# Hypersonic-cpu/DSP-AudioRecLabs

Hardware: NVIDIA B200
Metric: audio-seconds processed/sec (features+endpoints+KNN) (higher is better)
Workload: dtype i16->f32/f64

## Files before the change

dsp_audioreclabs_b200/csrc/capi.cu:

```cuda
#include <cmath>
#include <cstdarg>
#include <cstdio>
#include <cstdlib>
#include <cstring>
#include <string>
#include <vector>

#include "kernels.cuh"
#include "knn.cuh"
#include "mfcc_dtw.cuh"
#include "misc.cuh"

using namespace dsp;

namespace {

thread_local std::string g_err;

int fail(int code, const char* fmt, ...) {
  char buf[512];
  va_list ap;
  va_start(ap, fmt);
  vsnprintf(buf, sizeof buf, fmt, ap);
  va_end(ap);
// ... 779 lines not shown
  if (rc) return rc;
  CU(cudaMemcpyAsync(mean, dm, sizeof(double) * d, cudaMemcpyDeviceToHost, c->stream));
  CU(cudaMemcpyAsync(std, ds, sizeof(double) * d, cudaMemcpyDeviceToHost, c->stream));
  if (out) CU(cudaMemcpyAsync(out, dy, sizeof(double) * (size_t)n * d, cudaMemcpyDeviceToHost, c->stream));
  CU(cudaStreamSynchronize(c->stream));
  return DSP_OK;
}

static void knn_release(dsp_knn* k) {
  DevBuf* all[] = {&k->train64, &k->train32, &k->labels, &k->tnorm, &k->cand_idx, &k->cand_worst, &k->qnorm,
                   &k->redo_list, &k->redo_count, &k->nbr_label, &k->q, &k->o_idx, &k->o_dist, &k->o_lab,
                   &k->tpacked, &k->tnorm_dense, &k->qpacked, &k->qnorm_chunk, &k->dense_flags, &k->part_d, &k->part_i,
                   &k->tc_train, &k->tc_train_rows, &k->tc_q, &k->tc_flags, &k->refine_list, &k->refine_thr, &k->surv_count, &k->surv_rows, &k->thr0,
                   &k->prune_perm, &k->prune_geom, &k->prune_box, &k->prune_ws, &k->prune_bound};
  for (DevBuf* b : all) b->release();
}

int dsp_knn_fit_device(dsp_context* c, const double* train, const int32_t* labels, int64_t n, int32_t d, int32_t k,
                       int64_t index_base, dsp_knn** out) {
  if (!c || !out || n < 1 || d < 1 || k < 1 || !train || !labels) return fail(DSP_ERR_INVALID, "bad argument");
  if (k > kKnnMaxK) return fail(DSP_ERR_UNSUPPORTED, "n_neighbors > %d is not supported", kKnnMaxK);
  if (n > INT32_MAX) return fail(DSP_ERR_UNSUPPORTED, "more than 2^31 train rows per shard");
  CU(cudaSetDevice(c->device));
  dsp_knn* h = new dsp_knn();
  h->ctx = c; h->n = n; h->d = d; h->k = k; h->index_base = index_base; h->dp = knn_padded_dim(d);
  auto bail = [&](int code) { knn_release(h); delete h; return code; };
  if (h->train64.ensure(sizeof(double) * (size_t)n * d) != cudaSuccess || h->labels.ensure(sizeof(int32_t) * (size_t)n) != cudaSuccess ||
      h->tnorm.ensure(64) != cudaSuccess || h->redo_count.ensure(64) != cudaSuccess)
    return bail(fail(DSP_ERR_NOMEM, "device allocation failed"));
  cudaMemcpyAsync(h->train64.p, train, sizeof(double) * (size_t)n * d, cudaMemcpyDeviceToDevice, c->stream);
  cudaMemcpyAsync(h->labels.p, labels, sizeof(int32_t) * (size_t)n, cudaMemcpyDeviceToDevice, c->stream);
  if (h->dp) {
    if (h->train32.ensure(sizeof(float) * (size_t)n * h->dp) != cudaSuccess) return bail(fail(DSP_ERR_NOMEM, "device allocation failed"));
    cudaError_t e = knn_pack(h->train64.as<double>(), n, d, h->dp, h->train32.as<float>(), h->tnorm.as<float>(), c->stream);
    c->launches++;
    if (e != cudaSuccess) return bail(fail(DSP_ERR_CUDA, "knn_pack: %s", cudaGetErrorString(e)));
    cudaMemcpyAsync(&h->tnorm_max, h->tnorm.p, sizeof(float), cudaMemcpyDeviceToHost, c->stream);
  }
  int tc_flags[2] = {0, 1};
  if (h->dp == 16 && n >= 64 && k < kKnnCand && std::getenv("DSP_KNN_NO_TC16") == nullptr) {
    std::vector<double> host((size_t)n * d);
    if (cudaMemcpyAsync(host.data(), h->train64.p, sizeof(double) * host.size(), cudaMemcpyDeviceToHost, c->stream) != cudaSuccess ||
        cudaStreamSynchronize(c->stream) != cudaSuccess)
      return bail(fail(DSP_ERR_CUDA, "knn fit: %s", cudaGetErrorString(cudaGetLastError())));
    KnnPrunePlan plan;
    knn_prune_plan(host.data(), n, d, plan);
    h->prune_tiles = (int64_t)plan.slack.size();
    const size_t box = sizeof(double) * plan.lo.size();
    if (h->tc_train.ensure(knn_tc16_packed_bytes(n, false)) != cudaSuccess || h->tc_flags.ensure(64) != cudaSuccess ||
        h->prune_perm.ensure(sizeof(int) * (size_t)n) != cudaSuccess || h->prune_geom.ensure(sizeof(KnnPruneGeom)) != cudaSuccess ||
        h->prune_box.ensure(2 * box + sizeof(double) * plan.slack.size()) != cudaSuccess)
      return bail(fail(DSP_ERR_NOMEM, "device allocation failed"));
    unsigned char* pb = h->prune_box.as<unsigned char>();
    cudaMemcpyAsync(h->prune_perm.p, plan.perm.data(), sizeof(int) * (size_t)n, cudaMemcpyHostToDevice, c->stream);
    cudaMemcpyAsync(h->prune_geom.p, &plan.geom, sizeof(KnnPruneGeom), cudaMemcpyHostToDevice, c->stream);
    cudaMemcpyAsync(pb, plan.lo.data(), box, cudaMemcpyHostToDevice, c->stream);
    cudaMemcpyAsync(pb + box, plan.hi.data(), box, cudaMemcpyHostToDevice, c->stream);
    cudaMemcpyAsync(pb + 2 * box, plan.slack.data(), sizeof(double) * plan.slack.size(), cudaMemcpyHostToDevice, c->stream);
    if (h->tc_train_rows.ensure(knn_tc16_packed_bytes(n, false)) != cudaSuccess) return bail(fail(DSP_ERR_NOMEM, "device allocation failed"));
    cudaError_t e = knn_tc16_pack(h->train64.as<double>(), n, d, false, h->tc_train_rows.p, nullptr, h->tc_flags.as<int>(), c->stream);
    if (e == cudaSuccess)
      e = knn_tc16_pack(h->train64.as<double>(), n, d, false, h->tc_train.p, nullptr, h->tc_flags.as<int>(), c->stream,
                        h->prune_perm.as<int>());
    c->launches++;
    if (e != cudaSuccess) return bail(fail(DSP_ERR_CUDA, "knn_tc16_pack: %s", cudaGetErrorString(e)));
    cudaMemcpyAsync(tc_flags, h->tc_flags.p, sizeof tc_flags, cudaMemcpyDeviceToHost, c->stream);
    if (cudaStreamSynchronize(c->stream) != cudaSuccess)
      return bail(fail(DSP_ERR_CUDA, "knn fit: %s", cudaGetErrorString(cudaGetLastError())));
  }
  int dense_flags[2] = {0, 0};
  if (!h->dp && d <= kKnnDenseMaxDim && std::getenv("DSP_KNN_NO_DENSE") == nullptr) {
    if (h->tpacked.ensure(knn_dense_packed_bytes(n, d, true)) != cudaSuccess ||
        h->tnorm_dense.ensure(sizeof(float) * (size_t)knn_dense_padded_rows(n, true)) != cudaSuccess ||
        h->dense_flags.ensure(64) != cudaSuccess)
      return bail(fail(DSP_ERR_NOMEM, "device allocation failed"));
    cudaError_t e = knn_dense_pack(h->train64.as<double>(), n, d, true, h->tpacked.p, h->tnorm_dense.as<float>(), INFINITY,
                                   h->dense_flags.as<int>(), true, c->stream);
    c->launches++;
    if (e != cudaSuccess) return bail(fail(DSP_ERR_CUDA, "knn_dense_pack: %s", cudaGetErrorString(e)));
    cudaMemcpyAsync(dense_flags, h->dense_flags.p, sizeof dense_flags, cudaMemcpyDeviceToHost, c->stream);
  }
  cudaError_t e = cudaStreamSynchronize(c->stream);
  if (e != cudaSuccess) return bail(fail(DSP_ERR_CUDA, "knn fit: %s", cudaGetErrorString(e)));
  h->tc16 = h->tc_train.p && tc_flags[1] == 0;
  if (h->tpacked.p) {
    std::memcpy(&h->tnorm_max, &dense_flags[0], sizeof(float));
    h->dense = dense_flags[1] == 0;
  }
  *out = h;
  return DSP_OK;
}

int dsp_knn_fit_host(dsp_context* c, const double* train, const int32_t* labels, int64_t n, int32_t d, int32_t k,
                     int64_t index_base, dsp_knn** out) {
  if (!c || !out || n < 1 || d < 1 || k < 1 || !train || !labels) return fail(DSP_ERR_INVALID, "bad argument");
  if (k > kKnnMaxK) return fail(DSP_ERR_UNSUPPORTED, "n_neighbors > %d is not supported", kKnnMaxK);
  CU(cudaSetDevice(c->device));
  OneShot os(c);
  double* dt = os.dev<double>((size_t)n * d);
  int32_t* dl = os.dev<int32_t>((size_t)n);
  if (!dt || !dl) return fail(DSP_ERR_NOMEM, "device allocation failed");
  CU(cudaMemcpyAsync(dt, train, sizeof(double) * (size_t)n * d, cudaMemcpyHostToDevice, c->stream));
  CU(cudaMemcpyAsync(dl, labels, sizeof(int32_t) * (size_t)n, cudaMemcpyHostToDevice, c->stream));
  return dsp_knn_fit_device(c, dt, dl, n, d, k, index_base, out);
}

int dsp_knn_free(dsp_knn* k) {
  if (!k) return DSP_OK;
  cudaSetDevice(k->ctx->device);
  cudaStreamSynchronize(k->ctx->stream);
  knn_release(k);
  delete k;
  return DSP_OK;
}

int dsp_knn_topk_device(dsp_knn* h, const double* q, int64_t m, int64_t* nbr_idx, double* nbr_sqdist, int32_t* nbr_label) {
  return dsp_knn_topk_bounded_device(h, q, m, nullptr, nbr_idx, nbr_sqdist, nbr_label);
}

int dsp_knn_topk_bounded_device(dsp_knn* h, const double* q, int64_t m, const double* bound, int64_t* nbr_idx, double* nbr_sqdist,
                                int32_t* nbr_label) {
  if (!h || m < 0 || (!q && m)) return fail(DSP_ERR_INVALID, "bad argument");
  if (m == 0) return DSP_OK;
  if (m > INT32_MAX) return fail(DSP_ERR_UNSUPPORTED, "more than 2^31 queries per call");
  dsp_context* c = h->ctx;
  CU(cudaSetDevice(c->device));
  CU(h->redo_list.ensure(sizeof(int32_t) * (size_t)m));
  const unsigned long long* prune_kept = nullptr;
  int64_t prune_visits = 0;
  if (h->dp) {
    CU(h->cand_idx.ensure(sizeof(int) * (size_t)m * kKnnCand));
    CU(h->cand_worst.ensure(sizeof(float) * (size_t)m));
    CU(h->qnorm.ensure(sizeof(float) * (size_t)m));
    double err_rel = (double)(h->d + 4) * 1.1920929e-7, err_floor = 0.0;
    float qnorm_limit = 0.f;
    const float* thr0 = nullptr;
    const double* rerank_bound = nullptr;
    if (h->tc16) {
      CU(h->tc_q.ensure(knn_tc16_packed_bytes(m, true)));
      int* qflags = h->tc_flags.as<int>() + 4;
      err_rel = knn_dense_err_rel(16);
      err_floor = 1.0;
      qnorm_limit = knn_tc16_max_norm();
      Tc16Work work;
      const void* tpacked = h->tc_train_rows.p;
      const bool prune = c->knn_prune && knn_tc16_padded_rows(m, true) / kTc16UnitQueries * h->prune_tiles <= INT32_MAX;
      if (prune) {
        CU(h->prune_ws.ensure(knn_prune_scratch_bytes(m, h->n)));
        CU(h->prune_bound.ensure(sizeof(double) * (size_t)m));
        CU(h->thr0.ensure(sizeof(float) * (size_t)m));
        const unsigned char* pb = h->prune_box.as<unsigned char>();
        const size_t box = sizeof(double) * (size_t)h->prune_tiles * h->d;
        CU(knn_prune_prepare(q, m, h->n, h->d, h->k, h->train64.as<double>(), h->prune_geom.as<KnnPruneGeom>(), h->prune_perm.as<int>(),
                             (const double*)pb, (const double*)(pb + box), (const double*)(pb + 2 * box), h->tc_train.p, h->tc_q.p,
                             h->qnorm.as<float>(), qflags, bound, h->prune_bound.as<double>(), h->cand_idx.as<int>(),
                             h->cand_worst.as<float>(), h->prune_ws.p, c->knn_prune == 1, c->sm_count, c->stream, work));
        tpacked = h->tc_train.p;
        rerank_bound = h->prune_bound.as<double>();
        prune_kept = work.kept;
        prune_visits = knn_tc16_padded_rows(m, true) / kTc16UnitQueries * h->prune_tiles;
        CU(knn_bound_thresholds(rerank_bound, h->qnorm.as<float>(), m, err_rel, err_floor, h->thr0.as<float>(), c->stream));
        thr0 = h->thr0.as<float>();
        c->launches += 12;
      } else {
        CU(knn_tc16_pack(q, m, h->d, true, h->tc_q.p, h->qnorm.as<float>(), qflags, c->stream));
      }
      if (bound && !prune) {
        CU(h->thr0.ensure(sizeof(float) * (size_t)m));
        CU(knn_bound_thresholds(bound, h->qnorm.as<float>(), m, err_rel, err_floor, h->thr0.as<float>(), c->stream));
        thr0 = h->thr0.as<float>();
        rerank_bound = bound;
        c->launches += 1;
      }
      CU(knn_tc16_filter(h->tc_q.p, tpacked, m, h->n, h->k, qflags, h->cand_idx.as<int>(), h->cand_worst.as<float>(),
                         c->sm_count, c->stream, thr0, work));
      c->launches += 2;
    } else {
      CU(knn_scan(h->dp, h->train32.as<float>(), h->n, q, m, h->d, h->cand_idx.as<int>(), h->cand_worst.as<float>(),
                  h->qnorm.as<float>(), nullptr, c->stream));
      c->launches += 1;
    }
    const int refine_cap = (h->dp == 16 && h->k < kKnnCand) ? (int)std::min<int64_t>(m, 65536) : 0;
    h->refine_cap = refine_cap;
    if (refine_cap) {
      CU(h->refine_list.ensure(sizeof(int32_t) * (size_t)refine_cap));
      CU(h->refine_thr.ensure(sizeof(float) * (size_t)refine_cap));
      CU(h->surv_count.ensure(sizeof(int32_t) * (size_t)refine_cap));
      CU(h->surv_rows.ensure(sizeof(int32_t) * (size_t)refine_cap * knn_refine_survivor_cap()));
    }
    CU(knn_rerank(h->train64.as<double>(), h->train32.as<float>(), h->dp, h->n, q, m, h->d, h->k, h->index_base,
                  h->labels.as<int32_t>(), h->cand_idx.as<int>(), h->cand_worst.as<float>(), h->qnorm.as<float>(),
                  h->tnorm_max, err_rel, err_floor, nbr_idx, nbr_sqdist, nbr_label, h->redo_list.as<int32_t>(),
                  h->redo_count.as<int32_t>(), c->stream, refine_cap ? h->refine_list.as<int32_t>() : nullptr,
                  h->refine_thr.as<float>(), refine_cap, qnorm_limit, rerank_bound, thr0, bound && thr0));
    c->launches += 1;
    if (refine_cap) {
      CU(knn_refine(h->train64.as<double>(), h->train32.as<float>(), h->dp, h->n, q, h->d, h->k, h->index_base,
                    h->labels.as<int32_t>(), h->refine_list.as<int32_t>(), h->refine_thr.as<float>(), refine_cap,
                    h->surv_count.as<int32_t>(), h->surv_rows.as<int32_t>(), h->redo_count.as<int32_t>(),
                    h->redo_list.as<int32_t>(), nbr_idx, nbr_sqdist, nbr_label, c->sm_count, c->stream, bound && thr0));
      c->launches += 2;
    }
  } else if (h->dense) {
    h->refine_cap = 0;
    CU(h->cand_idx.ensure(sizeof(int) * (size_t)m * kKnnCand));
    CU(h->cand_worst.ensure(sizeof(float) * (size_t)m));
    CU(h->qnorm.ensure(sizeof(float) * (size_t)m));
    const int64_t chunk = std::min<int64_t>(m, kKnnDenseQueryChunk);
    CU(h->qpacked.ensure(knn_dense_packed_bytes(chunk, h->d, false)));
    CU(h->qnorm_chunk.ensure(sizeof(float) * (size_t)knn_dense_padded_rows(chunk, false)));
    CU(h->dense_flags.ensure(64));
    for (int64_t q0 = 0; q0 < m; q0 += chunk) {
      const int64_t mc = std::min<int64_t>(chunk, m - q0);
      CU(knn_dense_pack(q + q0 * h->d, mc, h->d, false, h->qpacked.p, h->qnorm_chunk.as<float>(), 0.f, h->dense_flags.as<int>(),
                        q0 == 0, c->stream));
      CU(cudaMemcpyAsync(h->qnorm.as<float>() + q0, h->qnorm_chunk.p, sizeof(float) * (size_t)mc, cudaMemcpyDeviceToDevice, c->stream));
      CU(knn_dense_scan(h->qpacked.p, h->tpacked.p, h->tnorm_dense.as<float>(), mc, h->n, h->d,
                        h->cand_idx.as<int>() + q0 * kKnnCand, h->cand_worst.as<float>() + q0, c->sm_count, c->stream));
      c->launches += 2;
    }
    int qflags[2] = {0, 0};
    CU(cudaMemcpyAsync(qflags, h->dense_flags.p, sizeof qflags, cudaMemcpyDeviceToHost, c->stream));
    CU(cudaStreamSynchronize(c->stream));
    const bool all_fit = qflags[1] == 0;
    if (all_fit) {
      CU(knn_rerank(h->train64.as<double>(), nullptr, 0, h->n, q, m, h->d, h->k, h->index_base,
                    h->labels.as<int32_t>(), h->cand_idx.as<int>(), h->cand_worst.as<float>(), h->qnorm.as<float>(),
                    h->tnorm_max, knn_dense_err_rel(h->d), 0.0, nbr_idx, nbr_sqdist, nbr_label, h->redo_list.as<int32_t>(),
                    h->redo_count.as<int32_t>(), c->stream));
    } else {
      CU(knn_redo_all(h->redo_list.as<int32_t>(), h->redo_count.as<int32_t>(), m, c->stream));
    }
    c->launches++;
  } else {
    h->refine_cap = 0;
    CU(knn_redo_all(h->redo_list.as<int32_t>(), h->redo_count.as<int32_t>(), m, c->stream));
    c->launches++;
  }
  CU(h->part_d.ensure(sizeof(double) * (size_t)knn_rescan_grid(c->sm_count) * kKnnMaxK));
  CU(h->part_i.ensure(sizeof(long long) * (size_t)knn_rescan_grid(c->sm_count) * kKnnMaxK));
  CU(knn_rescan(h->train64.as<double>(), h->n, q, h->d, h->k, h->index_base, h->labels.as<int32_t>(),
                h->redo_list.as<int32_t>(), h->redo_count.as<int32_t>(), nbr_idx, nbr_sqdist, nbr_label,
                c->sm_count, h->part_d.as<double>(), h->part_i.as<long long>(), (int)std::min<int64_t>(m, INT32_MAX), c->stream));
  c->launches++;
  if (std::getenv("DSP_KNN_DEBUG")) {
    int32_t cnt[4];
    cudaMemcpyAsync(cnt, h->redo_count.p, sizeof cnt, cudaMemcpyDeviceToHost, c->stream);
    cudaStreamSynchronize(c->stream);
    fprintf(stderr, "[knn] m=%lld n=%lld exhaustive=%d refined=%d refined->exhaustive=%d\n", (long long)m, (long long)h->n, cnt[0],
            std::min(cnt[1], h->refine_cap), cnt[2]);
    if (prune_kept) {
      unsigned long long kept = 0;
      cudaMemcpyAsync(&kept, prune_kept, sizeof kept, cudaMemcpyDeviceToHost, c->stream);
      cudaStreamSynchronize(c->stream);
      fprintf(stderr, "[knn] prune: tile visits kept=%llu of %lld (%s)\n", kept, (long long)prune_visits,
              c->knn_prune == 1 && kept > (unsigned long long)(0.85 * (double)prune_visits) ? "every tile walked" : "lists walked");
    }
  }
  return DSP_OK;
}

int dsp_mfcc_batch_host(dsp_context* c, const int16_t* samples, const int64_t* offsets, const int32_t* lengths,
                        const int32_t* seg_start, const int32_t* seg_end, int64_t n_utts, const dsp_mfcc_params* p,
                        const float* filterbank, const float* dct, const int64_t* mfcc_offsets, float* mfcc_out,
                        int32_t* n_frames_out) {
  if (!c || !p || n_utts < 0 || (n_utts && (!samples || !offsets || !seg_start || !seg_end || !filterbank || !dct || !mfcc_offsets || !mfcc_out)))
    return fail(DSP_ERR_INVALID, "bad argument");
  if (p->frame_length < 1 || p->frame_shift < 1 || p->n_mels < 1 || p->n_ceps < 1 || p->n_ceps > p->n_mels)
    return fail(DSP_ERR_INVALID, "bad MFCC geometry");
  if (p->n_fft < 32 || (p->n_fft & (p->n_fft - 1)) || p->n_fft < p->frame_length || p->n_fft > 16384)
    return fail(DSP_ERR_INVALID, "n_fft must be a power of two in [max(32, frame_length), 16384]");
  if (mfcc_smem_bytes(p->n_fft, p->n_mels) > kMaxSmemPerCta) return fail(DSP_ERR_UNSUPPORTED, "n_fft too large for shared memory");
  if (n_utts == 0) return DSP_OK;
  CU(cudaSetDevice(c->device));
  std::vector<double> w;
  int rc = host_window(p->window, p->frame_length, w);
  if (rc) return rc;
  std::vector<float> wf(w.begin(), w.end());
  const int n_bins = p->n_fft / 2 + 1;
  std::vector<float> tw((size_t)p->n_fft);
  for (int k = 0; k < p->n_fft / 2; ++k) {
    const double a = -2.0 * M_PI * (double)k / (double)p->n_fft;
    tw[2 * (size_t)k] = (float)std::cos(a); tw[2 * (size_t)k + 1] = (float)std::sin(a);
  }
  std::vector<int> range(2 * (size_t)p->n_mels);
  for (int m = 0; m < p->n_mels; ++m) {
    int lo = n_bins, hi = 0;
    for (int b = 0; b < n_bins; ++b) if (filterbank[(size_t)m * n_bins + b] != 0.f) { lo = std::min(lo, b); hi = std::max(hi, b + 1); }
    range[2 * (size_t)m] = std::min(lo, hi); range[2 * (size_t)m + 1] = hi;
  }
  const int64_t total_samples = lengths ? offsets[n_utts - 1] + lengths[n_utts - 1] : offsets[n_utts];
  int64_t span = 0;
  for (int64_t b = 0; b < n_utts; ++b) span = std::max<int64_t>(span, offsets[b] + (lengths ? lengths[b] : offsets[b + 1] - offsets[b]));
  const int64_t total_frames = mfcc_offsets[n_utts];
  (void)total_samples;
  OneShot os(c);
  int16_t* d_s = os.dev<int16_t>((size_t)span);
  int64_t* d_off = os.dev<int64_t>((size_t)n_utts + 1);
  int32_t* d_len = lengths ? os.dev<int32_t>((size_t)n_utts) : nullptr;
  int32_t* d_st = os.dev<int32_t>((size_t)n_utts);
  int32_t* d_en = os.dev<int32_t>((size_t)n_utts);
  float* d_w = os.dev<float>(wf.size());
  float* d_tw = os.dev<float>(tw.size());
  float* d_fb = os.dev<float>((size_t)p->n_mels * n_bins);
  int* d_rg = os.dev<int>(range.size());
  float* d_dct = os.dev<float>((size_t)p->n_ceps * p->n_mels);
  int64_t* d_mo = os.dev<int64_t>((size_t)n_utts + 1);
  float* d_out = os.dev<float>((size_t)std::max<int64_t>(total_frames, 1) * p->n_ceps);
  int32_t* d_nf = os.dev<int32_t>((size_t)n_utts);
  unsigned int* d_cnt = os.dev<unsigned int>(4);
  if (!d_s || !d_off || (lengths && !d_len) || !d_st || !d_en || !d_w || !d_tw || !d_fb || !d_rg || !d_dct || !d_mo || !d_out || !d_nf || !d_cnt)
    return fail(DSP_ERR_NOMEM, "device allocation failed");
  cudaStream_t st = c->stream;
  CU(cudaMemcpyAsync(d_s, samples, sizeof(int16_t) * (size_t)span, cudaMemcpyHostToDevice, st));
  CU(cudaMemcpyAsync(d_off, offsets, sizeof(int64_t) * ((size_t)n_utts + 1), cudaMemcpyHostToDevice, st));
  if (lengths) CU(cudaMemcpyAsync(d_len, lengths, sizeof(int32_t) * (size_t)n_utts, cudaMemcpyHostToDevice, st));
// ... 134 lines not shown
```

dsp_audioreclabs_b200/csrc/knn.cuh:

```cuda
#pragma once
#include <cuda_runtime.h>
#include <stdint.h>

#include <vector>

namespace dsp {

constexpr int kKnnCand = 8;
constexpr int kKnnMaxK = 16;

int knn_padded_dim(int d);
cudaError_t knn_pack(const double* train, int64_t n, int d, int dp, float* train32, float* tnorm_max,
                     cudaStream_t st);
cudaError_t knn_scan(int dp, const float* train32, int64_t n, const double* q, int64_t m, int d,
                     int* cand_idx, float* cand_worst, float* qnorm, const int* gate, cudaStream_t st);
cudaError_t knn_rerank(const double* train, const float* train32, int dp, int64_t n, const double* q,
                       int64_t m, int d, int k, int64_t index_base, const int32_t* labels,
                       const int* cand_idx, const float* cand_worst, const float* qnorm,
                       float tnorm_max_host, double err_rel, double err_floor, int64_t* nbr_idx, double* nbr_sqdist, int32_t* nbr_label,
                       int32_t* redo_list, int32_t* redo_count, cudaStream_t st, int32_t* refine_list = nullptr,
                       float* refine_thr = nullptr, int refine_cap = 0, float qnorm_limit = 0.f,
                       const double* bound = nullptr, const float* thr0 = nullptr, bool allow_short = true);
int knn_refine_survivor_cap();
cudaError_t knn_refine(const double* train, const float* train32, int dp, int64_t n, const double* q, int d, int k,
                       int64_t index_base, const int32_t* labels, const int32_t* refine_list, const float* refine_thr,
                       int refine_cap, int32_t* surv_count, int32_t* surv_rows, int32_t* counts, int32_t* redo_list,
                       int64_t* nbr_idx, double* nbr_sqdist, int32_t* nbr_label, int sm_count, cudaStream_t st,
                       bool allow_short = false);
cudaError_t knn_redo_all(int32_t* redo_list, int32_t* redo_count, int64_t m, cudaStream_t st);
cudaError_t knn_rescan(const double* train, int64_t n, const double* q, int d, int k, int64_t index_base,
                       const int32_t* labels, const int32_t* redo_list, const int32_t* redo_count,
                       int64_t* nbr_idx, double* nbr_sqdist, int32_t* nbr_label, int sm_count,
                       double* part_d, long long* part_i, int max_redo, cudaStream_t st);
int knn_rescan_grid(int sm_count);
cudaError_t knn_vote(const int32_t* nbr_label, int64_t m, int k, int32_t* out, cudaStream_t st);
cudaError_t knn_merge_vote(const double* cd, const int64_t* ci, const int32_t* cl, int r, int64_t m,
                           int k, int32_t* labels_out, int64_t* idx_out, double* dist_out,
                           cudaStream_t st);

float knn_tc16_max_norm();
int64_t knn_tc16_padded_rows(int64_t rows, bool query);
size_t knn_tc16_packed_bytes(int64_t rows, bool query);
constexpr int kTc16TileRows = 128;
constexpr int kTc16UnitQueries = 256;
cudaError_t knn_tc16_pack(const double* x, int64_t rows, int d, bool query, void* packed, float* norms, int* flags, cudaStream_t st,
                          const int* gather = nullptr);
struct Tc16Work {
  const int* tiles = nullptr;
  const int* tile_count = nullptr;
  int stride = 0;
  const int* unit_order = nullptr;
  int* counter = nullptr;
  const unsigned long long* kept = nullptr;
  unsigned long long kept_limit = 0;
  const int* qperm = nullptr;
  const int* tperm = nullptr;
};
cudaError_t knn_tc16_filter(const void* qpacked, const void* tpacked, int64_t m, int64_t n, int k, const int* qflags, int* cand_idx,
                            float* cand_worst, int sm_count, cudaStream_t st, const float* thr0 = nullptr, const Tc16Work& work = Tc16Work());

constexpr int kPruneMaxDim = 15;
constexpr int kPruneSeedTiles = 4;
struct KnnPruneGeom {
  int d;
  double mean[kPruneMaxDim];
  double axis[kPruneMaxDim][kPruneMaxDim];
  double key_lo[3], key_scale[3];
};
struct KnnPrunePlan {
  KnnPruneGeom geom;
  std::vector<int> perm;
  std::vector<double> lo, hi, slack;
};
void knn_prune_plan(const double* train, int64_t n, int d, KnnPrunePlan& plan);
size_t knn_prune_scratch_bytes(int64_t m, int64_t n);
cudaError_t knn_prune_prepare(const double* q, int64_t m, int64_t n, int d, int k, const double* train, const KnnPruneGeom* geom,
                              const int* tperm, const double* tile_lo, const double* tile_hi, const double* tile_slack, const void* tpacked,
                              void* qpacked, float* qnorm, int* qflags, const double* caller_bound, double* bound, int* cand_idx,
                              float* cand_worst, void* scratch, bool auto_fallback, int sm_count, cudaStream_t st, Tc16Work& work);
cudaError_t knn_bound_thresholds(const double* bound, const float* qnorm, int64_t m, double err_rel, double err_floor, float* thr0,
                                 cudaStream_t st);

int knn_dense_kblocks(int d);
int64_t knn_dense_padded_rows(int64_t rows, bool train);
size_t knn_dense_packed_bytes(int64_t rows, int d, bool train);
cudaError_t knn_dense_pack(const double* x, int64_t rows, int d, bool train, void* packed, float* norms, float pad_norm,
                           int* flags, bool reset_flags, cudaStream_t st);
cudaError_t knn_dense_scan(const void* qpacked, const void* tpacked, const float* tnorm, int64_t m, int64_t n, int d,
                           int* cand_idx, float* cand_worst, int sm_count, cudaStream_t st);
inline double knn_dense_err_rel(int d) { return (3.0 * d / 16.0 + 32.0) * 2.384185791015625e-07; }

}
```

dsp_audioreclabs_b200/csrc/knn_tc16.cu:

```cuda
#include <cuda_fp16.h>

#include <algorithm>
#include <climits>
#include <cmath>
#include <cstring>
#include <numeric>

#include <cub/block/block_scan.cuh>
#include <cub/device/device_radix_sort.cuh>

#include "kernels.cuh"
#include "knn.cuh"
#include "ptx.cuh"

namespace dsp {

namespace {

constexpr int kRows = 128;
constexpr int kK = 16;
constexpr int kPlaneBytes = kRows * kK * 2;
constexpr int kTileBytes = 2 * kPlaneBytes;
constexpr int kUnitQ = 2 * kRows;
constexpr int kQBufBytes = 2 * kTileBytes;
// ... 208 lines not shown
      for (int c = 0; c < kKnnCand; ++c) { l_cd[c * kEpiThreads] = INFINITY; l_ci[c * kEpiThreads] = -1; }
      const int64_t q_own = (int64_t)u * kUnitQ + h * kRows + lg * 32 + lane;
      const int64_t q_idx = q_own < m ? (w.qperm ? (int64_t)w.qperm[q_own] : q_own) : -1;
      const float thr_cap = (thr0 && q_idx >= 0) ? thr0[q_idx] : INFINITY;
      float thr = thr_cap;
      auto process = [&](const uint32_t* v, int idx0) {
        const float s0 = min8(v), s1 = min8(v + 8), s2 = min8(v + 16), s3 = min8(v + 24);
        if (fminf(fminf(s0, s1), fminf(s2, s3)) < thr) {
#define DSP_TC16_GROUP(g, sg)                                                                                                     \
          if (sg < thr)                                                                                                          \
            thr = fminf(thr_cap, tc16_slow8<kC>(__uint_as_float(v[8 * g]), __uint_as_float(v[8 * g + 1]), __uint_as_float(v[8 * g + 2]), \
                                 __uint_as_float(v[8 * g + 3]), __uint_as_float(v[8 * g + 4]), __uint_as_float(v[8 * g + 5]),        \
                                 __uint_as_float(v[8 * g + 6]), __uint_as_float(v[8 * g + 7]), idx0 + 8 * g, thr, l_cd, l_ci));
          DSP_TC16_GROUP(0, s0) DSP_TC16_GROUP(1, s1) DSP_TC16_GROUP(2, s2) DSP_TC16_GROUP(3, s3)
#undef DSP_TC16_GROUP
        }
        __syncwarp();
      };
      uint32_t va[32], vb[32];
      int row_next = cnt > 0 ? tile_row(0) : 0;
      for (int tb = 0; tb < cnt; ++tb) {
        const int base = row_next + half * 64;
        if (tb + 1 < cnt) row_next = tile_row(tb + 1);
        mbar_wait(&acc_full[as], aph);
        tc_fence_after();
        const uint32_t col = (uint32_t)((as * 2 + h) * kRows + half * 64);
        tmem_ld32(lane_addr + col, va);
        tmem_ld32(lane_addr + col + 32, vb);
        tmem_ld_wait();
        tc_fence_before();
        __syncwarp();
        if (lane == 0) mbar_arrive(&acc_empty[as]);
        if (++as == kAccStages) { as = 0; aph ^= 1u; }
        process(va, base);
        process(vb, base + 32);
      }
      const int pair_bar = 1 + lg + 4 * h;
      bar_sync(pair_bar, 64);
      if (half == 0) {
        float cd[kC]; int ci[kC];
#pragma unroll
        for (int c = 0; c < kC; ++c) { cd[c] = l_cd[c * kEpiThreads]; ci[c] = l_ci[c * kEpiThreads]; }
#pragma unroll
        for (int b = 0; b < kC; ++b) {
          float d = l_cd[b * kEpiThreads + 128]; int i = l_ci[b * kEpiThreads + 128];
#pragma unroll
          for (int c = 0; c < kC; ++c) {
            if (d < cd[c]) { const float td = cd[c]; const int ti = ci[c]; cd[c] = d; ci[c] = i; d = td; i = ti; }
          }
        }
#pragma unroll
        for (int c = 0; c < kC; ++c) { l_cd[c * kEpiThreads] = cd[c]; l_ci[c * kEpiThreads] = ci[c]; }
      }
      if (half == 0 && q_idx >= 0) {
#pragma unroll
        for (int c = 0; c < kKnnCand; ++c) {
          const int i = c < kC ? l_ci[c * kEpiThreads] : -1;
          cand_idx[q_idx * kKnnCand + c] = (i < 0 || !w.tperm) ? i : (i < n ? w.tperm[i] : -1);
        }
        cand_worst[q_idx] = l_cd[(kC - 1) * kEpiThreads];
      }
      bar_sync(pair_bar, 64);
    }
  }
  tc_fence_before();
  __syncthreads();
  if (warp == 1) {
    tc_fence_after();
    tmem_dealloc(tmem_base, kTmemCols);
  }
}


constexpr int kPruneThreads = kUnitQ;
constexpr double kPruneRel = 1e-9;
constexpr double kPruneSlack = 1e-13;

__device__ __forceinline__ double prune_project(const double* __restrict__ x, const KnnPruneGeom* __restrict__ g, int d, int na,
                                                double* __restrict__ p) {
  double c[kPruneMaxDim];
  double l1 = 0.0;
#pragma unroll
  for (int j = 0; j < kPruneMaxDim; ++j) { c[j] = j < d ? x[j] - g->mean[j] : 0.0; l1 += fabs(c[j]); }
#pragma unroll
  for (int a = 0; a < kPruneMaxDim; ++a) {
    if (a >= na) break;
    double s = 0.0;
    for (int j = 0; j < d; ++j) s += c[j] * g->axis[a][j];
    p[a] = s;
  }
  return l1;
}

__global__ void knn_prune_keys_kernel(const double* __restrict__ q, int64_t m, const KnnPruneGeom* __restrict__ g,
                                      unsigned* __restrict__ keys, int* __restrict__ vals) {
  const int64_t i = (int64_t)blockIdx.x * blockDim.x + threadIdx.x;
  if (i >= m) return;
  const int d = g->d, na = d < 3 ? d : 3;
  double p[kPruneMaxDim];
  prune_project(q + i * d, g, d, na, p);
  unsigned code = 0;
  for (int a = 0; a < na; ++a) {
    const double t = (p[a] - g->key_lo[a]) * g->key_scale[a];
    const unsigned v = t >= 0.0 ? (t < 1023.0 ? (unsigned)t : 1023u) : 0u;
#pragma unroll
    for (int b = 0; b < 10; ++b) code |= ((v >> b) & 1u) << (3 * b + 2 - a);
  }
  keys[i] = code;
  vals[i] = (int)i;
}

__device__ __forceinline__ double block_max(double v, double* sh) {
  v = warp_reduce(v, [](double a, double b) { return fmax(a, b); });
  __syncthreads();
  if ((threadIdx.x & 31) == 0) sh[threadIdx.x >> 5] = v;
  __syncthreads();
  double r = sh[0];
  for (int w = 1; w < kPruneThreads / 32; ++w) r = fmax(r, sh[w]);
  return r;
}

__global__ void __launch_bounds__(kPruneThreads)
knn_prune_unit_box_kernel(const double* __restrict__ q, int64_t m, const KnnPruneGeom* __restrict__ g, const int* __restrict__ qperm,
                          const float* __restrict__ qnorm, float qnorm_limit, double* __restrict__ ulo, double* __restrict__ uhi,
                          double* __restrict__ uslack) {
  __shared__ double s_lo[kPruneThreads / 32][kPruneMaxDim], s_hi[kPruneThreads / 32][kPruneMaxDim], s_red[kPruneThreads / 32];
  const int u = blockIdx.x, d = g->d, w = threadIdx.x >> 5, lane = threadIdx.x & 31;
  const int64_t pos = (int64_t)u * kUnitQ + threadIdx.x;
  const int64_t qi = pos < m ? qperm[pos] : -1;
  const bool valid = qi >= 0 && qnorm[qi] <= qnorm_limit;
  double p[kPruneMaxDim], l1 = 0.0;
  if (valid) l1 = prune_project(q + qi * d, g, d, d, p);
#pragma unroll
  for (int a = 0; a < kPruneMaxDim; ++a) {
    if (a >= d) break;
    const double lo = warp_reduce(valid ? p[a] : INFINITY, [](double x, double y) { return fmin(x, y); });
    const double hi = warp_reduce(valid ? p[a] : -INFINITY, [](double x, double y) { return fmax(x, y); });
    if (lane == 0) { s_lo[w][a] = lo; s_hi[w][a] = hi; }
  }
  const double l1max = block_max(l1, s_red);
  if (threadIdx.x < d) {
    double lo = INFINITY, hi = -INFINITY;
    for (int ww = 0; ww < kPruneThreads / 32; ++ww) { lo = fmin(lo, s_lo[ww][threadIdx.x]); hi = fmax(hi, s_hi[ww][threadIdx.x]); }
    ulo[(int64_t)u * d + threadIdx.x] = lo;
    uhi[(int64_t)u * d + threadIdx.x] = hi;
  }
  if (threadIdx.x == 0) uslack[u] = kPruneSlack * (1.0 + l1max);
}

__device__ __forceinline__ bool less_dt(double da, int ta, double db, int tb) { return da < db || (da == db && ta < tb); }

__global__ void __launch_bounds__(kPruneThreads)
knn_prune_seed_kernel(int t_tiles, int d, const double* __restrict__ ulo, const double* __restrict__ uhi, const double* __restrict__ tlo,
                      const double* __restrict__ thi, int S, int* __restrict__ seed, int* __restrict__ seed_cnt) {
  __shared__ double s_d[kPruneThreads / 32];
  __shared__ int s_t[kPruneThreads / 32];
  __shared__ int s_win;
  const int u = blockIdx.x, w = threadIdx.x >> 5, lane = threadIdx.x & 31;
  double c[kPruneMaxDim];
  for (int a = 0; a < d; ++a) c[a] = 0.5 * (ulo[(int64_t)u * d + a] + uhi[(int64_t)u * d + a]);
  double bd[kPruneSeedTiles];
  int bt[kPruneSeedTiles];
#pragma unroll
  for (int s = 0; s < kPruneSeedTiles; ++s) { bd[s] = INFINITY; bt[s] = INT_MAX; }
  for (int t = threadIdx.x; t < t_tiles; t += kPruneThreads) {
    double dd = 0.0;
    for (int a = 0; a < d; ++a) { const double x = c[a] - 0.5 * (tlo[(int64_t)t * d + a] + thi[(int64_t)t * d + a]); dd += x * x; }
    if (!(dd < INFINITY)) dd = INFINITY;
    int s = kPruneSeedTiles - 1;
    if (!less_dt(dd, t, bd[s], bt[s])) continue;
    while (s > 0 && less_dt(dd, t, bd[s - 1], bt[s - 1])) { bd[s] = bd[s - 1]; bt[s] = bt[s - 1]; --s; }
    bd[s] = dd; bt[s] = t;
  }
  for (int r = 0; r < S; ++r) {
    double md = bd[0];
    int mt = bt[0];
#pragma unroll
    for (int o = 16; o > 0; o >>= 1) {
      const double od = __shfl_xor_sync(0xffffffffu, md, o);
      const int ot = __shfl_xor_sync(0xffffffffu, mt, o);
      if (less_dt(od, ot, md, mt)) { md = od; mt = ot; }
    }
    if (lane == 0) { s_d[w] = md; s_t[w] = mt; }
    __syncthreads();
    if (threadIdx.x == 0) {
      for (int ww = 1; ww < kPruneThreads / 32; ++ww) if (less_dt(s_d[ww], s_t[ww], md, mt)) { md = s_d[ww]; mt = s_t[ww]; }
      s_win = mt;
      seed[(int64_t)u * S + r] = mt;
    }
    __syncthreads();
    if (bt[0] == s_win) {
#pragma unroll
      for (int s = 0; s + 1 < kPruneSeedTiles; ++s) { bd[s] = bd[s + 1]; bt[s] = bt[s + 1]; }
      bd[kPruneSeedTiles - 1] = INFINITY; bt[kPruneSeedTiles - 1] = INT_MAX;
    }
  }
  if (threadIdx.x == 0) seed_cnt[u] = S;
}

__global__ void __launch_bounds__(kPruneThreads)
knn_prune_bound_kernel(const double* __restrict__ train, const double* __restrict__ q, int64_t m, int d, int k,
                       const int* __restrict__ qperm, const int* __restrict__ cand_idx, const float* __restrict__ qnorm, float qnorm_limit,
                       const double* __restrict__ caller_bound, double* __restrict__ bound, double* __restrict__ unit_rad) {
  __shared__ double s_red[kPruneThreads / 32];
  const int u = blockIdx.x;
  const int64_t pos = (int64_t)u * kUnitQ + threadIdx.x;
  const int64_t qi = pos < m ? qperm[pos] : -1;
  const bool valid = qi >= 0 && qnorm[qi] <= qnorm_limit;
  double U = INFINITY;
  if (qi >= 0) {
    double best[kKnnCand];
    int nb = 0;
    for (int c = 0; c < kKnnCand; ++c) {
      const int i = cand_idx[qi * kKnnCand + c];
      if (i < 0) continue;
      double dd = 0.0;
      for (int j = 0; j < d; ++j) { const double x = q[qi * d + j] - train[(int64_t)i * d + j]; dd += x * x; }
      int s = nb++;
      while (s > 0 && dd < best[s - 1]) { best[s] = best[s - 1]; --s; }
      best[s] = dd;
    }
    if (nb >= k) U = best[k - 1];
    if (caller_bound) U = fmin(U, caller_bound[qi]);
    bound[qi] = U;
  }
  const double any = block_max(valid ? 1.0 : 0.0, s_red);
  const double r = block_max(valid ? U : -INFINITY, s_red);
  if (threadIdx.x == 0) unit_rad[u] = any > 0.0 ? r : INFINITY;
}

__global__ void __launch_bounds__(kPruneThreads)
knn_prune_list_kernel(int t_tiles, int d, const double* __restrict__ ulo, const double* __restrict__ uhi, const double* __restrict__ uslack,
                      const double* __restrict__ unit_rad, const double* __restrict__ tlo, const double* __restrict__ thi,
                      const double* __restrict__ tslack, int* __restrict__ tiles, int* __restrict__ count, int* __restrict__ unit_ids,
                      unsigned long long* __restrict__ kept) {
  using Scan = cub::BlockScan<int, kPruneThreads>;
  __shared__ typename Scan::TempStorage scan_tmp;
  __shared__ double s_lo[kPruneMaxDim], s_hi[kPruneMaxDim];
  const int u = blockIdx.x;
  if (threadIdx.x < d) { s_lo[threadIdx.x] = ulo[(int64_t)u * d + threadIdx.x]; s_hi[threadIdx.x] = uhi[(int64_t)u * d + threadIdx.x]; }
  __syncthreads();
  const double lim = unit_rad[u] * (1.0 + kPruneRel), sl_u = uslack[u];
  int run = 0;
  for (int base = 0; base < t_tiles; base += kPruneThreads) {
    const int t = base + threadIdx.x;
    int keep = 0;
    if (t < t_tiles) {
      const double sl = sl_u + tslack[t];
      double lb = 0.0;
      for (int a = 0; a < d; ++a) {
        const double gap = fmax(tlo[(int64_t)t * d + a] - s_hi[a], s_lo[a] - thi[(int64_t)t * d + a]) - sl;
        if (gap > 0.0) lb += gap * gap;
      }
      keep = lb <= lim;
    }
    int at, total;
    Scan(scan_tmp).ExclusiveSum(keep, at, total);
    if (keep) tiles[(int64_t)u * t_tiles + run + at] = t;
    run += total;
    __syncthreads();
  }
  if (threadIdx.x == 0) {
    count[u] = run;
    unit_ids[u] = u;
    atomicAdd(kept, (unsigned long long)run);
  }
}

}

float knn_tc16_max_norm() { return 8192.f; }
int64_t knn_tc16_padded_rows(int64_t rows, bool query) { const int b = query ? kUnitQ : kRows; return (rows + b - 1) / b * b; }
size_t knn_tc16_packed_bytes(int64_t rows, bool query) { return (size_t)(knn_tc16_padded_rows(rows, query) / kRows) * kTileBytes; }

cudaError_t knn_tc16_pack(const double* x, int64_t rows, int d, bool query, void* packed, float* norms, int* flags, cudaStream_t st,
                          const int* gather) {
  cudaMemsetAsync(flags, 0, 2 * sizeof(int), st);
  const int64_t rp = knn_tc16_padded_rows(rows, query);
  if (rp == 0) return cudaSuccess;
  knn_tc16_pack_kernel<<<(unsigned)((rp + 127) / 128), 128, 0, st>>>(x, rows, rp, d, query, static_cast<unsigned char*>(packed), norms,
                                                                    flags, knn_tc16_max_norm(), gather);
  return cudaGetLastError();
}

cudaError_t knn_tc16_filter(const void* qpacked, const void* tpacked, int64_t m, int64_t n, int k, const int* qflags, int* cand_idx,
                            float* cand_worst, int sm_count, cudaStream_t st, const float* thr0, const Tc16Work& work) {
  if (m == 0) return cudaSuccess;
  const int units = (int)(knn_tc16_padded_rows(m, true) / kUnitQ), t_tiles = (int)(knn_tc16_padded_rows(n, false) / kRows);
  auto fn = k <= 3 ? knn_tc16_filter_kernel<5> : knn_tc16_filter_kernel<kKnnCand>;
  cudaError_t e = cudaFuncSetAttribute(fn, cudaFuncAttributeMaxDynamicSharedMemorySize, (int)kTcSmem);
  if (e != cudaSuccess) return e;
  const int grid = units < sm_count ? units : sm_count;
  if (work.counter) cudaMemsetAsync(work.counter, 0, sizeof(int), st);
  fn<<<grid, kTcThreads, kTcSmem, st>>>(static_cast<const unsigned char*>(qpacked), static_cast<const unsigned char*>(tpacked), m, (int)n,
                                        units, t_tiles, qflags, cand_idx, cand_worst, thr0, work);
  return cudaGetLastError();
}

}

namespace dsp {

namespace {

void jacobi_eigen(int d, double a[kPruneMaxDim][kPruneMaxDim], double v[kPruneMaxDim][kPruneMaxDim]) {
  for (int i = 0; i < d; ++i)
    for (int j = 0; j < d; ++j) v[i][j] = i == j ? 1.0 : 0.0;
  for (int sweep = 0; sweep < 100; ++sweep) {
    double off = 0.0, diag = 0.0;
    for (int p = 0; p < d; ++p) {
      diag += a[p][p] * a[p][p];
      for (int q = p + 1; q < d; ++q) off += a[p][q] * a[p][q];
    }
    if (!(off > 1e-32 * diag)) break;
    for (int p = 0; p < d; ++p)
      for (int q = p + 1; q < d; ++q) {
        if (a[p][q] == 0.0) continue;
        const double theta = (a[q][q] - a[p][p]) / (2.0 * a[p][q]);
        const double t = std::fabs(theta) > 1e150 ? 0.5 / theta : (theta >= 0 ? 1.0 : -1.0) / (std::fabs(theta) + std::sqrt(theta * theta + 1.0));
        const double c = 1.0 / std::sqrt(t * t + 1.0), s = t * c;
        for (int k = 0; k < d; ++k) { const double x = a[k][p], y = a[k][q]; a[k][p] = c * x - s * y; a[k][q] = s * x + c * y; }
        for (int k = 0; k < d; ++k) { const double x = a[p][k], y = a[q][k]; a[p][k] = c * x - s * y; a[q][k] = s * x + c * y; }
        for (int k = 0; k < d; ++k) { const double x = v[k][p], y = v[k][q]; v[k][p] = c * x - s * y; v[k][q] = s * x + c * y; }
      }
  }
}

struct PruneScratch {
  unsigned* keys[2];
  int* vals[2];
  void* sort_tmp;
  size_t sort_bytes;
  double *ulo, *uhi, *uslack, *rad;
  int *seed, *seed_cnt, *tiles, *count[2], *ids[2], *counter;
  unsigned long long* kept;
};

size_t prune_layout(int64_t m, int64_t n, unsigned char* base, PruneScratch& s) {
  const int64_t units = knn_tc16_padded_rows(m, true) / kUnitQ, t_tiles = knn_tc16_padded_rows(n, false) / kRows;
  size_t b1 = 0, b2 = 0;
  cub::DeviceRadixSort::SortPairs(nullptr, b1, (const unsigned*)nullptr, (unsigned*)nullptr, (const int*)nullptr, (int*)nullptr, (int)m, 0, 30);
  cub::DeviceRadixSort::SortPairsDescending(nullptr, b2, (const int*)nullptr, (int*)nullptr, (const int*)nullptr, (int*)nullptr, (int)units);
  s.sort_bytes = std::max(b1, b2);
  size_t off = 0;
  auto take = [&](size_t bytes) { void* p = base ? base + off : nullptr; off += (bytes + 255) / 256 * 256; return p; };
  for (int i = 0; i < 2; ++i) { s.keys[i] = (unsigned*)take(4 * (size_t)m); s.vals[i] = (int*)take(4 * (size_t)m); }
  s.sort_tmp = take(s.sort_bytes);
  s.ulo = (double*)take(8 * (size_t)units * kPruneMaxDim);
  s.uhi = (double*)take(8 * (size_t)units * kPruneMaxDim);
  s.uslack = (double*)take(8 * (size_t)units);
  s.rad = (double*)take(8 * (size_t)units);
  s.seed = (int*)take(4 * (size_t)units * kPruneSeedTiles);
  s.seed_cnt = (int*)take(4 * (size_t)units);
  s.tiles = (int*)take(4 * (size_t)units * t_tiles);
  for (int i = 0; i < 2; ++i) { s.count[i] = (int*)take(4 * (size_t)units); s.ids[i] = (int*)take(4 * (size_t)units); }
  s.counter = (int*)take(4);
  s.kept = (unsigned long long*)take(8);
  return off;
}

}

void knn_prune_plan(const double* x, int64_t n, int d, KnnPrunePlan& plan) {
  KnnPruneGeom& g = plan.geom;
  std::memset(&g, 0, sizeof g);
  g.d = d;
  for (int j = 0; j < d; ++j) {
    double s = 0.0;
    for (int64_t i = 0; i < n; ++i) s += x[i * d + j];
    g.mean[j] = s / (double)n;
  }
  double cov[kPruneMaxDim][kPruneMaxDim] = {}, vec[kPruneMaxDim][kPruneMaxDim];
  for (int64_t i = 0; i < n; ++i)
    for (int p = 0; p < d; ++p)
      for (int q = p; q < d; ++q) cov[p][q] += (x[i * d + p] - g.mean[p]) * (x[i * d + q] - g.mean[q]);
  for (int p = 0; p < d; ++p)
    for (int q = p; q < d; ++q) cov[q][p] = cov[p][q] /= (double)n;
  jacobi_eigen(d, cov, vec);
  int order[kPruneMaxDim];
  std::iota(order, order + d, 0);
  std::stable_sort(order, order + d, [&](int a, int b) { return cov[a][a] > cov[b][b]; });
  for (int a = 0; a < d; ++a)
    for (int j = 0; j < d; ++j) g.axis[a][j] = vec[j][order[a]];
  std::vector<double> pr((size_t)n * d), l1((size_t)n);
  for (int64_t i = 0; i < n; ++i) {
    double c[kPruneMaxDim], s1 = 0.0;
    for (int j = 0; j < d; ++j) { c[j] = x[i * d + j] - g.mean[j]; s1 += std::fabs(c[j]); }
    l1[(size_t)i] = s1;
    for (int a = 0; a < d; ++a) {
      double s = 0.0;
      for (int j = 0; j < d; ++j) s += c[j] * g.axis[a][j];
      pr[(size_t)i * d + a] = s;
    }
  }
  const int64_t t_tiles = knn_tc16_padded_rows(n, false) / kRows;
  plan.perm.resize((size_t)n);
  std::iota(plan.perm.begin(), plan.perm.end(), 0);
  int* perm = plan.perm.data();
  std::vector<std::pair<int64_t, int64_t>> stack{{0, t_tiles}};
  while (!stack.empty()) {
    const auto [t0, t1] = stack.back();
    stack.pop_back();
    if (t1 - t0 < 2) continue;
    const int64_t r0 = t0 * kRows, r1 = std::min<int64_t>(t1 * kRows, n), tm = t0 + (t1 - t0) / 2, rm = tm * kRows;
    int axis = 0;
    double widest = -1.0;
    for (int a = 0; a < d; ++a) {
      double lo = INFINITY, hi = -INFINITY;
      for (int64_t r = r0; r < r1; ++r) { const double v = pr[(size_t)perm[r] * d + a]; lo = std::min(lo, v); hi = std::max(hi, v); }
      if (hi - lo > widest) { widest = hi - lo; axis = a; }
    }
    std::nth_element(perm + r0, perm + rm, perm + r1, [&](int i, int j) {
      const double a = pr[(size_t)i * d + axis], b = pr[(size_t)j * d + axis];
      return a < b || (a == b && i < j);
    });
    stack.push_back({t0, tm});
    stack.push_back({tm, t1});
  }
  plan.lo.assign((size_t)t_tiles * d, INFINITY);
  plan.hi.assign((size_t)t_tiles * d, -INFINITY);
  plan.slack.assign((size_t)t_tiles, 0.0);
  for (int64_t r = 0; r < n; ++r) {
    const int64_t t = r / kRows, i = perm[r];
    for (int a = 0; a < d; ++a) {
      plan.lo[(size_t)t * d + a] = std::min(plan.lo[(size_t)t * d + a], pr[(size_t)i * d + a]);
      plan.hi[(size_t)t * d + a] = std::max(plan.hi[(size_t)t * d + a], pr[(size_t)i * d + a]);
    }
    plan.slack[(size_t)t] = std::max(plan.slack[(size_t)t], kPruneSlack * (1.0 + l1[(size_t)i]));
  }
  for (int a = 0; a < 3 && a < d; ++a) {
    double lo = INFINITY, hi = -INFINITY;
    for (int64_t t = 0; t < t_tiles; ++t) { lo = std::min(lo, plan.lo[(size_t)t * d + a]); hi = std::max(hi, plan.hi[(size_t)t * d + a]); }
    g.key_lo[a] = lo;
    g.key_scale[a] = hi > lo ? 1024.0 / (hi - lo) : 0.0;
  }
}

size_t knn_prune_scratch_bytes(int64_t m, int64_t n) {
  PruneScratch s;
  return prune_layout(m, n, nullptr, s);
}

cudaError_t knn_prune_prepare(const double* q, int64_t m, int64_t n, int d, int k, const double* train, const KnnPruneGeom* geom,
                              const int* tperm, const double* tile_lo, const double* tile_hi, const double* tile_slack, const void* tpacked,
                              void* qpacked, float* qnorm, int* qflags, const double* caller_bound, double* bound, int* cand_idx,
                              float* cand_worst, void* scratch, bool auto_fallback, int sm_count, cudaStream_t st, Tc16Work& work) {
  if (m == 0) return cudaSuccess;
  PruneScratch s;
  prune_layout(m, n, static_cast<unsigned char*>(scratch), s);
  const int units = (int)(knn_tc16_padded_rows(m, true) / kUnitQ), t_tiles = (int)(knn_tc16_padded_rows(n, false) / kRows);
  const float limit = knn_tc16_max_norm();
  knn_prune_keys_kernel<<<(unsigned)((m + 255) / 256), 256, 0, st>>>(q, m, geom, s.keys[0], s.vals[0]);
  size_t bytes = s.sort_bytes;
  cudaError_t e = cub::DeviceRadixSort::SortPairs(s.sort_tmp, bytes, s.keys[0], s.keys[1], s.vals[0], s.vals[1], (int)m, 0, 30, st);
  if (e != cudaSuccess) return e;
  const int* qperm = s.vals[1];
  if ((e = knn_tc16_pack(q, m, d, true, qpacked, qnorm, qflags, st, qperm)) != cudaSuccess) return e;
  knn_prune_unit_box_kernel<<<units, kPruneThreads, 0, st>>>(q, m, geom, qperm, qnorm, limit, s.ulo, s.uhi, s.uslack);
  const int S = std::min(kPruneSeedTiles, t_tiles);
  knn_prune_seed_kernel<<<units, kPruneThreads, 0, st>>>(t_tiles, d, s.ulo, s.uhi, tile_lo, tile_hi, S, s.seed, s.seed_cnt);
  Tc16Work seed;
  seed.tiles = s.seed; seed.tile_count = s.seed_cnt; seed.stride = S;
  seed.qperm = qperm; seed.tperm = tperm;
  if ((e = knn_tc16_filter(qpacked, tpacked, m, n, k, qflags, cand_idx, cand_worst, sm_count, st, nullptr, seed)) != cudaSuccess) return e;
  knn_prune_bound_kernel<<<units, kPruneThreads, 0, st>>>(train, q, m, d, k, qperm, cand_idx, qnorm, limit, caller_bound, bound, s.rad);
  cudaMemsetAsync(s.kept, 0, sizeof(unsigned long long), st);
  knn_prune_list_kernel<<<units, kPruneThreads, 0, st>>>(t_tiles, d, s.ulo, s.uhi, s.uslack, s.rad, tile_lo, tile_hi, tile_slack, s.tiles,
                                                         s.count[0], s.ids[0], s.kept);
  bytes = s.sort_bytes;
  e = cub::DeviceRadixSort::SortPairsDescending(s.sort_tmp, bytes, s.count[0], s.count[1], s.ids[0], s.ids[1], units, 0, 32, st);
  if (e != cudaSuccess) return e;
  work = Tc16Work();
  work.tiles = s.tiles; work.tile_count = s.count[0]; work.stride = t_tiles;
  work.unit_order = s.ids[1]; work.counter = s.counter;
  work.kept = s.kept;
  work.kept_limit = auto_fallback ? (unsigned long long)(0.85 * (double)units * (double)t_tiles) : ~0ull;
  work.qperm = qperm; work.tperm = tperm;
  return cudaGetLastError();
}

}
```

Baseline: 20.19 million.

## Compute seed-tile candidates inside prune bound kernel instead of tensor-core filter pass

Drops the separate tensor-core filter launch over the seed tiles. The prune bound kernel now stages each unit's seed-tile training rows in shared memory as fp32 and has every query thread compute its own top-8 candidates by scalar FMA distance before refining them in double precision. This removes a launch and the cand_idx/cand_worst round trip through global memory. In exchange, the seed search runs on CUDA cores with a per-thread insertion sort rather than on tensor cores, and each block now holds a larger shared-memory footprint.

New measurement: 20.05 million, median of 6. Within noise of the previous version (-0.7%).

```diff
diff --git a/dsp_audioreclabs_b200/csrc/capi.cu b/dsp_audioreclabs_b200/csrc/capi.cu
--- a/dsp_audioreclabs_b200/csrc/capi.cu
+++ b/dsp_audioreclabs_b200/csrc/capi.cu
@@ -955,16 +955,16 @@
         const unsigned char* pb = h->prune_box.as<unsigned char>();
         const size_t box = sizeof(double) * (size_t)h->prune_tiles * h->d;
         CU(knn_prune_prepare(q, m, h->n, h->d, h->k, h->train64.as<double>(), h->prune_geom.as<KnnPruneGeom>(), h->prune_perm.as<int>(),
-                             (const double*)pb, (const double*)(pb + box), (const double*)(pb + 2 * box), h->tc_train.p, h->tc_q.p,
-                             h->qnorm.as<float>(), qflags, bound, h->prune_bound.as<double>(), h->cand_idx.as<int>(),
-                             h->cand_worst.as<float>(), h->prune_ws.p, c->knn_prune == 1, c->sm_count, c->stream, work));
+                             (const double*)pb, (const double*)(pb + box), (const double*)(pb + 2 * box), h->tc_q.p,
+                             h->qnorm.as<float>(), qflags, bound, h->prune_bound.as<double>(), h->prune_ws.p, c->knn_prune == 1,
+                             c->stream, work));
         tpacked = h->tc_train.p;
         rerank_bound = h->prune_bound.as<double>();
         prune_kept = work.kept;
         prune_visits = knn_tc16_padded_rows(m, true) / kTc16UnitQueries * h->prune_tiles;
         CU(knn_bound_thresholds(rerank_bound, h->qnorm.as<float>(), m, err_rel, err_floor, h->thr0.as<float>(), c->stream));
         thr0 = h->thr0.as<float>();
-        c->launches += 12;
+        c->launches += 11;
       } else {
         CU(knn_tc16_pack(q, m, h->d, true, h->tc_q.p, h->qnorm.as<float>(), qflags, c->stream));
       }
diff --git a/dsp_audioreclabs_b200/csrc/knn.cuh b/dsp_audioreclabs_b200/csrc/knn.cuh
--- a/dsp_audioreclabs_b200/csrc/knn.cuh
+++ b/dsp_audioreclabs_b200/csrc/knn.cuh
@@ -75,9 +75,9 @@
 void knn_prune_plan(const double* train, int64_t n, int d, KnnPrunePlan& plan);
 size_t knn_prune_scratch_bytes(int64_t m, int64_t n);
 cudaError_t knn_prune_prepare(const double* q, int64_t m, int64_t n, int d, int k, const double* train, const KnnPruneGeom* geom,
-                              const int* tperm, const double* tile_lo, const double* tile_hi, const double* tile_slack, const void* tpacked,
-                              void* qpacked, float* qnorm, int* qflags, const double* caller_bound, double* bound, int* cand_idx,
-                              float* cand_worst, void* scratch, bool auto_fallback, int sm_count, cudaStream_t st, Tc16Work& work);
+                              const int* tperm, const double* tile_lo, const double* tile_hi, const double* tile_slack,
+                              void* qpacked, float* qnorm, int* qflags, const double* caller_bound, double* bound, void* scratch,
+                              bool auto_fallback, cudaStream_t st, Tc16Work& work);
 cudaError_t knn_bound_thresholds(const double* bound, const float* qnorm, int64_t m, double err_rel, double err_floor, float* thr0,
                                  cudaStream_t st);
 
diff --git a/dsp_audioreclabs_b200/csrc/knn_tc16.cu b/dsp_audioreclabs_b200/csrc/knn_tc16.cu
--- a/dsp_audioreclabs_b200/csrc/knn_tc16.cu
+++ b/dsp_audioreclabs_b200/csrc/knn_tc16.cu
@@ -384,7 +384,7 @@
 
 __global__ void __launch_bounds__(kPruneThreads)
 knn_prune_seed_kernel(int t_tiles, int d, const double* __restrict__ ulo, const double* __restrict__ uhi, const double* __restrict__ tlo,
-                      const double* __restrict__ thi, int S, int* __restrict__ seed, int* __restrict__ seed_cnt) {
+                      const double* __restrict__ thi, int S, int* __restrict__ seed) {
   __shared__ double s_d[kPruneThreads / 32];
   __shared__ int s_t[kPruneThreads / 32];
   __shared__ int s_win;
@@ -427,25 +427,68 @@
       bd[kPruneSeedTiles - 1] = INFINITY; bt[kPruneSeedTiles - 1] = INT_MAX;
     }
   }
-  if (threadIdx.x == 0) seed_cnt[u] = S;
-}
-
+}
+
+constexpr int kSeedRows = kPruneSeedTiles * kRows;
 __global__ void __launch_bounds__(kPruneThreads)
-knn_prune_bound_kernel(const double* __restrict__ train, const double* __restrict__ q, int64_t m, int d, int k,
-                       const int* __restrict__ qperm, const int* __restrict__ cand_idx, const float* __restrict__ qnorm, float qnorm_limit,
-                       const double* __restrict__ caller_bound, double* __restrict__ bound, double* __restrict__ unit_rad) {
+knn_prune_bound_kernel(const double* __restrict__ train, const double* __restrict__ q, int64_t m, int n, int d, int k,
+                       const int* __restrict__ qperm, const int* __restrict__ tperm, const int* __restrict__ seed, int S,
+                       const float* __restrict__ qnorm, float qnorm_limit, const double* __restrict__ caller_bound,
+                       double* __restrict__ bound, double* __restrict__ unit_rad) {
+  __shared__ __align__(16) float s_t[kSeedRows][16];
+  __shared__ int s_row[kSeedRows];
   __shared__ double s_red[kPruneThreads / 32];
   const int u = blockIdx.x;
+  for (int r = threadIdx.x; r < S * kRows; r += kPruneThreads) {
+    const int64_t p = (int64_t)seed[(int64_t)u * S + r / kRows] * kRows + r % kRows;
+    const int row = p < n ? tperm[p] : -1;
+    s_row[r] = row;
+#pragma unroll
+    for (int j = 0; j < 16; ++j) s_t[r][j] = (row >= 0 && j < d) ? (float)train[(int64_t)row * d + j] : 0.f;
+  }
+  __syncthreads();
   const int64_t pos = (int64_t)u * kUnitQ + threadIdx.x;
   const int64_t qi = pos < m ? qperm[pos] : -1;
   const bool valid = qi >= 0 && qnorm[qi] <= qnorm_limit;
   double U = INFINITY;
   if (qi >= 0) {
+    float qf[16];
+#pragma unroll
+    for (int j = 0; j < 16; ++j) qf[j] = j < d ? (float)q[qi * d + j] : 0.f;
+    float bd[kKnnCand];
+    int bi[kKnnCand];
+#pragma unroll
+    for (int c = 0; c < kKnnCand; ++c) { bd[c] = INFINITY; bi[c] = -1; }
+    for (int r0 = 0; r0 < S * kRows; r0 += 4) {
+      float dd[4];
+#pragma unroll
+      for (int i = 0; i < 4; ++i) {
+        const float4* t = reinterpret_cast<const float4*>(s_t[r0 + i]);
+        float a = 0.f;
+#pragma unroll
+        for (int v = 0; v < 4; ++v) {
+          const float4 x = t[v];
+          const float x0 = qf[4 * v] - x.x, x1 = qf[4 * v + 1] - x.y, x2 = qf[4 * v + 2] - x.z, x3 = qf[4 * v + 3] - x.w;
+          a = fmaf(x0, x0, a); a = fmaf(x1, x1, a); a = fmaf(x2, x2, a); a = fmaf(x3, x3, a);
+        }
+        dd[i] = s_row[r0 + i] < 0 ? INFINITY : a;
+      }
+#pragma unroll
+      for (int i = 0; i < 4; ++i) {
+        if (dd[i] < bd[kKnnCand - 1]) {
+          float x = dd[i]; int xi = r0 + i;
+#pragma unroll
+          for (int c = 0; c < kKnnCand; ++c) {
+            if (x < bd[c]) { const float tx = bd[c]; const int ti = bi[c]; bd[c] = x; bi[c] = xi; x = tx; xi = ti; }
+          }
+        }
+      }
+    }
     double best[kKnnCand];
     int nb = 0;
     for (int c = 0; c < kKnnCand; ++c) {
-      const int i = cand_idx[qi * kKnnCand + c];
-      if (i < 0) continue;
+      if (bi[c] < 0) continue;
+      const int i = s_row[bi[c]];
       double dd = 0.0;
       for (int j = 0; j < d; ++j) { const double x = q[qi * d + j] - train[(int64_t)i * d + j]; dd += x * x; }
       int s = nb++;
@@ -564,7 +607,7 @@
   void* sort_tmp;
   size_t sort_bytes;
   double *ulo, *uhi, *uslack, *rad;
-  int *seed, *seed_cnt, *tiles, *count[2], *ids[2], *counter;
+  int *seed, *tiles, *count[2], *ids[2], *counter;
   unsigned long long* kept;
 };
 
@@ -583,7 +626,6 @@
   s.uslack = (double*)take(8 * (size_t)units);
   s.rad = (double*)take(8 * (size_t)units);
   s.seed = (int*)take(4 * (size_t)units * kPruneSeedTiles);
-  s.seed_cnt = (int*)take(4 * (size_t)units);
   s.tiles = (int*)take(4 * (size_t)units * t_tiles);
   for (int i = 0; i < 2; ++i) { s.count[i] = (int*)take(4 * (size_t)units); s.ids[i] = (int*)take(4 * (size_t)units); }
   s.counter = (int*)take(4);
@@ -674,9 +716,9 @@
 }
 
 cudaError_t knn_prune_prepare(const double* q, int64_t m, int64_t n, int d, int k, const double* train, const KnnPruneGeom* geom,
-                              const int* tperm, const double* tile_lo, const double* tile_hi, const double* tile_slack, const void* tpacked,
-                              void* qpacked, float* qnorm, int* qflags, const double* caller_bound, double* bound, int* cand_idx,
-                              float* cand_worst, void* scratch, bool auto_fallback, int sm_count, cudaStream_t st, Tc16Work& work) {
+                              const int* tperm, const double* tile_lo, const double* tile_hi, const double* tile_slack,
+                              void* qpacked, float* qnorm, int* qflags, const double* caller_bound, double* bound, void* scratch,
+                              bool auto_fallback, cudaStream_t st, Tc16Work& work) {
   if (m == 0) return cudaSuccess;
   PruneScratch s;
   prune_layout(m, n, static_cast<unsigned char*>(scratch), s);
@@ -690,12 +732,9 @@
   if ((e = knn_tc16_pack(q, m, d, true, qpacked, qnorm, qflags, st, qperm)) != cudaSuccess) return e;
   knn_prune_unit_box_kernel<<<units, kPruneThreads, 0, st>>>(q, m, geom, qperm, qnorm, limit, s.ulo, s.uhi, s.uslack);
   const int S = std::min(kPruneSeedTiles, t_tiles);
-  knn_prune_seed_kernel<<<units, kPruneThreads, 0, st>>>(t_tiles, d, s.ulo, s.uhi, tile_lo, tile_hi, S, s.seed, s.seed_cnt);
-  Tc16Work seed;
-  seed.tiles = s.seed; seed.tile_count = s.seed_cnt; seed.stride = S;
-  seed.qperm = qperm; seed.tperm = tperm;
-  if ((e = knn_tc16_filter(qpacked, tpacked, m, n, k, qflags, cand_idx, cand_worst, sm_count, st, nullptr, seed)) != cudaSuccess) return e;
-  knn_prune_bound_kernel<<<units, kPruneThreads, 0, st>>>(train, q, m, d, k, qperm, cand_idx, qnorm, limit, caller_bound, bound, s.rad);
+  knn_prune_seed_kernel<<<units, kPruneThreads, 0, st>>>(t_tiles, d, s.ulo, s.uhi, tile_lo, tile_hi, S, s.seed);
+  knn_prune_bound_kernel<<<units, kPruneThreads, 0, st>>>(train, q, m, (int)n, d, k, qperm, tperm, s.seed, S, qnorm, limit, caller_bound,
+                                                          bound, s.rad);
   cudaMemsetAsync(s.kept, 0, sizeof(unsigned long long), st);
   knn_prune_list_kernel<<<units, kPruneThreads, 0, st>>>(t_tiles, d, s.ulo, s.uhi, s.uslack, s.rad, tile_lo, tile_hi, tile_slack, s.tiles,
                                                          s.count[0], s.ids[0], s.kept);
```
